# rapidsai/cuvs

Measured on AMD Instinct MI355X. Metric: QPS @ recall@10>=0.9, 100Mx128 fp32 IVF-PQ, batch=10k, higher is better.
Workload: dtype u8 codes, f16 LUT, f32 score; 1 GPU; IVF-PQ 100000000x128 fp32, pq_dim=64 pq_bits=8 n_lists=16384 n_probes=128 batch=10000 k=10; rows and held-out queries from bench.gen_rows (seed 1234 / 4321): Gaussian mixture of 65536 modes ~ N(0, I) in a 32-d latent space, spread 0.35 per mode, embedded in R^128 by a fixed random map + N(0, 0.03^2 I) - NOT SURVEY 8d's generator: the same step on that one is the top-level entry contract_corpus (--; parallelism=single GPU, lut_dtype=f16, internal_distance_dtype=f32

## Files before the change

cuvs_amd/csrc/common.hpp:

```cpp
#pragma once

#include <hip/hip_runtime.h>
#include <hip/hip_fp16.h>

#include <dlpack/dlpack.h>

#include <cstdarg>
#include <cstdint>
#include <cstdio>
#include <cstring>
#include <memory>
#include <stdexcept>
#include <string>
#include <chrono>
#include <vector>

namespace cuvs_amd {

struct error : public std::runtime_error {
  explicit error(const std::string& s) : std::runtime_error(s) {}
};

[[noreturn]] inline void fail(const char* file, int line, const char* fmt, ...)
{
// ... 15 lines not shown
#define HIP_TRY(expr)                                                                        \
  do {                                                                                       \
    hipError_t e__ = (expr);                                                                 \
    if (e__ != hipSuccess) {                                                                 \
      ::cuvs_amd::fail(__FILE__, __LINE__, "HIP error %d (%s) in %s", (int)e__,              \
                       hipGetErrorString(e__), #expr);                                       \
    }                                                                                        \
  } while (0)

std::string& last_error_text();

template <typename Fn>
int translate_exceptions(Fn&& fn)
{
  try {
    fn();
    return 1;
  } catch (const std::exception& e) {
    last_error_text() = e.what();
    return 0;
  } catch (...) {
    last_error_text() = "unknown exception";
    return 0;
  }
}

struct tuning {
  int pq_head_probes    = -1;
  int pq_scan2          = 1;
  int pq_scan3          = 1;
  int coarse_lowp       = 1;
  int pq_head_rows      = -1;
  int pq_overlap        = 1;
  int coarse_grouped    = 1;
  int pq_filter4        = 1;
  int flat_scan3        = 1;
  int flat_filter2      = 1;
  int flat_bound_head   = 1;
  int pq_wide           = 1;
  int pq_wide_heads     = 0;
  int pq_wide_blocks    = 1;
  bool pq_encode_plain  = false;
  int pq3_surv_cap      = 0;
  int pq_qcap           = 0;
  int scan_debug        = 0;
  int alloc_cache       = 1;
  bool shard_coarse_replicated = false;
  bool bf_fused = false, bf_no_threshold = false, bf_no_fused_filter = false;
  bool bf_host_flags = false;
  bool dist_old         = false;
  int tile_dbg          = 0;
  int flat_head_probes  = -1;
  int cagra_pq_lists = 0, cagra_pq_probes = 0, cagra_kpq = 0, cagra_rank_chunk = 0, prune_dbg = 0;
  bool cagra_auto_multi = false;
  int tiered_path       = 0;
  bool native_format    = false;
};
tuning load_tuning_from_env();

struct resources {
  tuning tune;
  int device              = 0;
  hipStream_t stream      = nullptr;
  bool owns_stream        = false;
  int num_cus             = 256;
  size_t lds_per_block    = 160 * 1024;
// ... 211 lines not shown
```

cuvs_amd/csrc/core.hip:

```cpp
#include <cuvs/version_config.h>
#include "common.hpp"

#include <cuvs/core/c_api.h>

#include "scratch_cache.hpp"

#include <algorithm>
#include <cstdlib>
#include <mutex>
#include <vector>

namespace cuvs_amd {

std::string& last_error_text()
{
  thread_local std::string text;
  return text;
}

namespace {

void* raw_alloc(resources& res, size_t bytes, bool* failed)
{
  void* p = nullptr;
  hipError_t e = res.pool != nullptr ? hipMallocFromPoolAsync(&p, bytes, res.pool, res.stream)
                                     : hipMallocAsync(&p, bytes, res.stream);
  if (e != hipSuccess) {
    (void)hipGetLastError();
    if (failed != nullptr) { *failed = true; return nullptr; }
    HIP_TRY(hipStreamSynchronize(res.stream));
    HIP_TRY(hipMalloc(&p, bytes));
  }
  return p;
}

void raw_free(void* stream_v, void* p)
{
  hipStream_t stream = static_cast<hipStream_t>(stream_v);
  hipError_t e = hipFreeAsync(p, stream);
  if (e != hipSuccess) {
    (void)hipGetLastError();
    (void)hipStreamSynchronize(stream);
    (void)hipFree(p);
  }
}

}

unsigned long long g_pq3_last_stats[6] = {0, 0, 0, 0, 0, 0};

static void flush_cache(scratch_cache& c)
{
  if (!c.caller_stream) { c.flush(raw_free); return; }
  bool drained = false;
  c.flush([&](void*, void* p) {
    if (!drained) { (void)hipDeviceSynchronize(); drained = true; }
    (void)hipFree(p);
    (void)hipGetLastError();
  });
}
void scratch_cache_flush(resources& res)
{
  if (res.cache != nullptr) flush_cache(*res.cache);
}

namespace {
std::mutex g_caches_mu;
std::vector<scratch_cache*> g_caches;
}
void scratch_cache_register(scratch_cache* c, bool add)
{
  std::lock_guard<std::mutex> lk(g_caches_mu);
  if (add) g_caches.push_back(c);
  else g_caches.erase(std::remove(g_caches.begin(), g_caches.end(), c), g_caches.end());
}
void scratch_cache_flush_all()
{
  {
    std::lock_guard<std::mutex> lk(g_caches_mu);
    for (scratch_cache* c : g_caches) flush_cache(*c);
  }
  (void)hipDeviceSynchronize();
// ... 63 lines not shown
  g_prof.push_back(r);
}
void profile_end(resources& res, const char* name)
{
  if (!g_prof_on) return;
  std::lock_guard<std::mutex> lk(g_prof_mu);
  for (auto it = g_prof.rbegin(); it != g_prof.rend(); ++it)
    if (it->name == name) { HIP_TRY(hipEventRecord(it->stop, res.stream)); return; }
}

static bool debug_switches_on()
{
#ifdef CUVS_AMD_NO_DEBUG_SWITCHES
  return false;
#else
  const char* g = getenv("CUVS_AMD_DEBUG_SWITCHES");
  return g != nullptr && g[0] == '1';
#endif
}

tuning load_tuning_from_env()
{
  tuning t;
  if (!debug_switches_on()) return t;
  auto geti = [](const char* name, int dflt) { const char* e = getenv(name); return e ? atoi(e) : dflt; };
  auto set  = [](const char* name) { return getenv(name) != nullptr; };
  t.pq_head_probes   = geti("CUVS_AMD_PQ_HEAD_PROBES", -1);
  t.pq_scan2         = geti("CUVS_AMD_PQ_SCAN2", 1);
  t.pq_scan3         = geti("CUVS_AMD_PQ_SCAN3", 1);
  t.pq_filter4       = geti("CUVS_AMD_PQ_FILTER4", 1);
  t.coarse_grouped   = geti("CUVS_AMD_COARSE_GROUPED", 1);
  t.pq_overlap       = geti("CUVS_AMD_PQ_OVERLAP", 1);
  t.pq_head_rows     = geti("CUVS_AMD_PQ_HEAD_ROWS", -1);
  t.coarse_lowp      = geti("CUVS_AMD_COARSE_LOWP", 1);
  t.flat_scan3       = geti("CUVS_AMD_FLAT_SCAN3", 1);
  t.flat_filter2     = geti("CUVS_AMD_FLAT_FILTER2", 1);
  t.flat_bound_head  = geti("CUVS_AMD_FLAT_BOUND_HEAD", 1);
  t.pq_wide          = geti("CUVS_AMD_PQ_WIDE", 1);
  t.pq_wide_heads    = geti("CUVS_AMD_PQ_WIDE_HEADS", 0);
  t.pq_wide_blocks   = geti("CUVS_AMD_PQ_WIDE_BLOCKS", 1);
  if (const char* e = getenv("CUVS_AMD_PQ_ENCODE")) t.pq_encode_plain = strcmp(e, "plain") == 0;
  t.pq3_surv_cap     = geti("CUVS_AMD_PQ3_SURV_CAP", 0);
  t.pq_qcap          = geti("CUVS_AMD_PQ_QCAP", 0);
  t.scan_debug       = geti("CUVS_AMD_SCAN_DEBUG", 0);
  t.alloc_cache      = geti("CUVS_AMD_ALLOC_CACHE", 1);
  t.shard_coarse_replicated = set("CUVS_AMD_SHARD_COARSE_REPLICATED");
  t.bf_fused           = set("CUVS_AMD_BF_FUSED");
  t.bf_no_threshold    = set("CUVS_AMD_BF_NO_THRESHOLD");
  t.bf_no_fused_filter = set("CUVS_AMD_BF_NO_FUSED_FILTER");
  t.bf_host_flags = set("CUVS_AMD_BF_HOST_FLAGS");
  t.dist_old           = set("CUVS_AMD_DIST_OLD");
  t.tile_dbg           = geti("CUVS_AMD_TILE_DBG", 0);
  t.flat_head_probes   = geti("CUVS_AMD_FLAT_HEAD_PROBES", -1);
  t.cagra_pq_lists     = geti("CUVS_AMD_CAGRA_PQ_LISTS", 0);
  t.cagra_pq_probes    = geti("CUVS_AMD_CAGRA_PQ_PROBES", 0);
  t.cagra_kpq          = geti("CUVS_AMD_CAGRA_KPQ", 0);
  t.cagra_rank_chunk   = geti("CUVS_AMD_CAGRA_RANK_CHUNK", 0);
  t.prune_dbg          = geti("CUVS_AMD_PRUNE_DBG", 0);
  if (const char* e = getenv("CUVS_AMD_CAGRA_AUTO")) t.cagra_auto_multi = e[0] == 'm';
  if (const char* e = getenv("CUVS_AMD_TIERED_PATH")) t.tiered_path = strcmp(e, "composed") == 0 ? 1 : (strcmp(e, "fused") == 0 ? 2 : 0);
  if (const char* e = getenv("CUVS_AMD_NATIVE_FORMAT")) t.native_format = e[0] == '1';
  return t;
}

}

// ... 201 lines not shown
}

cuvsError_t cuvsRMMMemoryResourceReset() { return CUVS_SUCCESS; }

cuvsError_t cuvsRMMHostAlloc(void** ptr, size_t bytes)
{
  return (cuvsError_t)translate_exceptions([=] {
    CUVS_EXPECTS(ptr != nullptr, "ptr is null");
    HIP_TRY(hipHostMalloc(ptr, bytes, hipHostMallocDefault));
  });
}

cuvsError_t cuvsRMMHostFree(void* ptr, size_t)
{
  return (cuvsError_t)translate_exceptions([=] { HIP_TRY(hipHostFree(ptr)); });
}

__attribute__((visibility("default"))) int cuvsAmdDebugSwitchesCompiledIn(void)
{
#ifdef CUVS_AMD_NO_DEBUG_SWITCHES
  return 0;
#else
  return 1;
#endif
}
__attribute__((visibility("default"))) void cuvsAmdIvfPqLastFilterStats(unsigned long long* out)
{
  for (int i = 0; i < 4; ++i) out[i] = cuvs_amd::g_pq3_last_stats[i];
}
__attribute__((visibility("default"))) void cuvsAmdIvfPqLastFilterStats6(unsigned long long* out)
{
  for (int i = 0; i < 6; ++i) out[i] = cuvs_amd::g_pq3_last_stats[i];
}
__attribute__((visibility("default"))) void cuvsAmdProfileEnable(int on) { g_prof_on = on != 0; }
__attribute__((visibility("default"))) int cuvsAmdProfileCollect(const char* name, double* total_ms)
{
  std::lock_guard<std::mutex> lk(g_prof_mu);
  int count = 0;
  double total = 0;
  std::vector<prof_rec> keep;
  for (auto& r : g_prof) {
    if (r.name == name) {
      if (hipEventSynchronize(r.stop) == hipSuccess) {
        float ms = 0;
        if (hipEventElapsedTime(&ms, r.start, r.stop) == hipSuccess) { total += ms; ++count; }
      }
      (void)hipEventDestroy(r.start);
      (void)hipEventDestroy(r.stop);
    } else {
      keep.push_back(r);
    }
  }
  g_prof.swap(keep);
  if (total_ms) *total_ms = total;
  return count;
}

cuvsError_t cuvsVersionGet(uint16_t* major, uint16_t* minor, uint16_t* patch)
{
  return (cuvsError_t)translate_exceptions([=] {
    CUVS_EXPECTS(major && minor && patch, "null output");
    *major = CUVS_VERSION_MAJOR; *minor = CUVS_VERSION_MINOR; *patch = CUVS_VERSION_PATCH;
  });
}

cuvsError_t cuvsMatrixCopy(cuvsResources_t res, DLManagedTensor* src_m, DLManagedTensor* dst_m)
// ... 46 lines not shown
```

cuvs_amd/csrc/ivf_pq_scan3.hip:

```cpp
#include "ivf_pq.hpp"
#include "ops.hpp"
#include "device_utils.hpp"
#include "ivf_common.hpp"
#include "pq_lut_math.hpp"
#include "ivf_pq_scan3.hpp"
#include "ivf_pq_filter_common.hpp"

#include <cfloat>
#include <cmath>
#include <cstring>
#include <mutex>
#include <type_traits>

namespace cuvs_amd {

namespace {

constexpr int kFThreads = 512;
constexpr int kFWaves   = kFThreads / 64;



__global__ void cb16_kernel(const float* __restrict__ pq_centers, uint32_t pq_dim, uint32_t pq_len, uint32_t book, float sc,
                            uint16_t* __restrict__ cb16)
// ... 1767 lines not shown
            } else {
              const float t = qq[e] - x[e4 * 4 + e];
              acc = __fmaf_rn(t, t, acc);
            }
          }
        }
      }
    }
    if (a.is_ip == 2) acc = acc / (sqrtf(qn2) * sqrtf(xn2));
    pool_append_wave(a, ok, q, pair, row, a.is_ip ? -acc : acc);
  }
}

struct head_params {
  const work_item* items;
  const uint32_t* item_begin;
  const uint32_t* item_end;
  uint32_t n_lists;
  uint32_t* xcd_ticket;
  const uint32_t* sorted_pairs;
  const float* rot_queries;
  const float* centers_rot;
  const float* pq_centers;
  const uint8_t* codes;
  const uint32_t* list_offsets;
  const uint32_t* list_sizes;
  float* out_d;
  uint32_t* out_i;
  uint32_t* query_kth;
  uint32_t n_probes, rot_dim, k, cap_rows, pq_dim, n_chunks, pq_len, book;
  int is_ip, per_cluster;
  int hcand;
  uint32_t row_limit;
  uint32_t one_shot;
  const uint32_t* filter_bits;
  const int64_t* indices;
  unsigned long long* stats;
};

static inline int head_cand(int k) { return k <= 128 ? 512 : 1024; }

template <int LUT, bool ACC_HALF, int NT>
__global__ __launch_bounds__(NT) __attribute__((amdgpu_waves_per_eu(4, 4))) void pq_head_kernel(const head_params a)
{
  constexpr bool LUT32 = LUT == 0 || (LUT == 2 && !ACC_HALF);
  using lut_t = std::conditional_t<LUT32, float, _Float16>;
  extern __shared__ __attribute__((aligned(16))) char smem[];
  lut_t* lut      = reinterpret_cast<lut_t*>(smem);
  float* rv       = reinterpret_cast<float*>(smem + (size_t)a.pq_dim * 256 * sizeof(lut_t));
  float* cv       = rv + 256;
  unsigned long long* min64 = reinterpret_cast<unsigned long long*>(cv + 256);
  int* ctrl       = reinterpret_cast<int*>(min64 + 2);
  work_item& cur  = *reinterpret_cast<work_item*>(ctrl + 8);
  uint32_t* tk    = reinterpret_cast<uint32_t*>(ctrl + 12);
  const int kHCand = a.hcand;
  uint2* cand     = reinterpret_cast<uint2*>(tk + NT);
  uint32_t* keys  = reinterpret_cast<uint32_t*>(cand + 2 * kHCand);
  static_assert(sizeof(work_item) == 16, "work_item");

  const int tid = threadIdx.x;
  const uint32_t item0   = (a.one_shot == 0u && a.item_begin) ? *a.item_begin : 0u;
  const uint32_t n_items = a.one_shot != 0u ? a.one_shot : *a.item_end - item0;
  const uint32_t xcd = blockIdx.x & 7u, chunk = (n_items + 7u) / 8u;
  const uint32_t share0 = min(n_items, xcd * chunk), share_len = min(chunk, n_items - share0);
  const work_item* share = a.items + item0 + share0;
  const uint4* codes16   = reinterpret_cast<const uint4*>(a.codes);
// ... 74 lines not shown
            p[j] = a.pq_centers[(size_t)((a.per_cluster ? L : sb) * a.pq_len + l) * a.book + code];
          }
#pragma unroll
          for (int j = 0; j < 4; ++j) {
            const uint32_t e = min(e0 + (uint32_t)j * NT, a.pq_dim * 256u - 1u), dd = (e >> 8) * a.pq_len + l;
            const float qv = rv[dd];
            if (!a.is_ip) {
              const float d = qv - p[j];
              v[j] = __fmaf_rn(d, d, v[j]);
            } else {
              v[j] = __fmaf_rn(-qv, cv[dd], v[j]);
              v[j] = __fmaf_rn(-qv, p[j], v[j]);
            }
          }
        }
#pragma unroll
        for (int j = 0; j < 4; ++j) {
          const uint32_t e = e0 + (uint32_t)j * NT;
          if (e >= a.pq_dim * 256u) break;
          float x = v[j];
          if constexpr (LUT == 2) x = fp8_round_trip<std::conditional_t<ACC_HALF, __half, float>>(x, a.is_ip != 0);
          if constexpr (LUT32) lut[e] = x; else lut[e] = to_lut_half(x);
        }
      }
    }
    if (tid == 0) ctrl[0] = 0;
    __syncthreads();
    phase(1);
    const int k = (int)a.k;
    int buf = 0;
    for (uint32_t c0 = 0; c0 < len; c0 += a.cap_rows) {
      const uint32_t clen = min(a.cap_rows, len - c0);
      uint32_t my_min = 0xffffffffu;
      for (uint32_t v = tid; v < clen; v += NT) {
        const uint32_t fr = base_row + c0 + v;
        const uint4* cp   = codes16 + ((size_t)(fr >> 6) * a.n_chunks) * 64 + (fr & 63u);
        float af    = 0.f;
        _Float16 ah = (_Float16)0.f;
        for (int c0c = 0; c0c < (int)a.n_chunks; c0c += 4) {
          uint4 cw[4];
#pragma unroll
          for (int c = 0; c < 4; ++c) cw[c] = cp[(size_t)min(c0c + c, (int)a.n_chunks - 1) * 64];
#pragma unroll
          for (int cc = 0; cc < 4; ++cc) {
            const int c = c0c + cc;
            if (c >= (int)a.n_chunks) break;
            const uint32_t ws[4] = {cw[cc].x, cw[cc].y, cw[cc].z, cw[cc].w};
            lut_t e[16];
#pragma unroll
            for (int b = 0; b < 16; ++b) e[b] = lut[((c * 16 + b) << 8) + ((ws[b >> 2] >> ((b & 3) * 8)) & 0xffu)];
            __builtin_amdgcn_sched_barrier(0);
#pragma unroll
            for (int b = 0; b < 16; ++b) {
              if constexpr (LUT32) af += e[b];
              else if constexpr (ACC_HALF) ah += e[b];
              else af += (float)e[b];
            }
          }
        }
        const float score = ACC_HALF ? (float)ah : af;
        bool keep = true;
        if (a.filter_bits != nullptr) {
          const int64_t sid = a.indices[fr];
          keep = ((a.filter_bits[sid >> 5] >> (sid & 31)) & 1u) != 0u;
        }
        const uint32_t key = keep ? float_to_key(score) : 0xffffffffu;
        keys[v] = key;
        my_min  = min(my_min, key);
      }
      const int gshift = k > 128 ? 0 : (k > 64 ? 1 : 2);
      if (gshift >= 1)
        my_min = min(my_min, (uint32_t)__builtin_amdgcn_update_dpp((int)my_min, (int)my_min, 0xb1, 0xf, 0xf, false));
      if (gshift == 2)
        my_min = min(my_min, (uint32_t)__builtin_amdgcn_update_dpp((int)my_min, (int)my_min, 0x4e, 0xf, 0xf, false));
      if ((tid & ((1 << gshift) - 1)) == 0) tk[tid >> gshift] = my_min;
      __syncthreads();
      phase(2);
      const int NGr   = NT >> gshift;
      const int k_c   = (int)min((uint32_t)k, clen);
      const int kept  = ctrl[0];
      if (tid < NGr) {
        const uint32_t mine = tk[tid];
        const uint4* tk4    = reinterpret_cast<const uint4*>(tk);
        int r = 0;
#pragma unroll 4
        for (int j = 0; j < NGr / 4; ++j) {
          const uint4 o = tk4[j];
          r += (o.x < mine || (o.x == mine && 4 * j + 0 < tid)) ? 1 : 0;
          r += (o.y < mine || (o.y == mine && 4 * j + 1 < tid)) ? 1 : 0;
          r += (o.z < mine || (o.z == mine && 4 * j + 2 < tid)) ? 1 : 0;
          r += (o.w < mine || (o.w == mine && 4 * j + 3 < tid)) ? 1 : 0;
        }
        if (r == k_c - 1) ctrl[1] = (int)mine;
        if (tid == 0) ctrl[2] = kept;
      }
      __syncthreads();
      const uint32_t tau = (uint32_t)ctrl[1];
      uint2* bc = cand + buf * kHCand;
      for (uint32_t i = tid; i < clen; i += NT) {
        const uint32_t key = keys[i];
        if (key <= tau && key != 0xffffffffu) {
          const int pos = atomicAdd(&ctrl[2], 1);
          if (pos < kHCand) bc[pos] = make_uint2(key, c0 + i);
        }
      }
      __syncthreads();
      int cnt = ctrl[2];
      if (cnt > kHCand) {
        unsigned long long last = 0ull;
        bool first = true;
        cnt = kept;
// ... 450 lines not shown
  hipLaunchKernelGGL(reset_flagged_kernel, dim3((unsigned)r.nq), dim3(256), 0, res.stream, r.qflag, r.nq, r.n_probes, r.k, r.head,
                     r.cand_d, r.cand_i);
  hipLaunchKernelGGL(fallback_items_kernel, dim3(grid * 4), dim3(256), 0, res.stream, r.sorted_pairs, r.pair_off, idx.n_lists,
                     r.probes, r.n_probes, r.qflag, static_cast<work_item*>(r.fb_items), r.counters, 0);
  profile_end(res, "pq_scan_kernel");
}

static size_t head_smem_fixed(const ivf_pq_index& idx, int lut_mode, bool acc_half, int nt, int k)
{
  const bool lut32 = lut_mode == 0 || (lut_mode == 2 && !acc_half);
  return (size_t)idx.pq_dim * 256 * (lut32 ? 4 : 2) + 2 * 256 * 4 + 16 + 32 + 16 + (size_t)nt * 4 + 4 * (size_t)head_cand(k) * 4;
}

void pq3_head_scan(resources& res, const ivf_pq_index& idx, const pq3_head& h)
{
  head_params a{};
  a.items = static_cast<const work_item*>(h.items); a.item_begin = h.item_begin; a.item_end = h.item_end; a.n_lists = idx.n_lists;
  a.xcd_ticket = h.xcd_ticket; a.sorted_pairs = h.sorted_pairs; a.rot_queries = h.rot_queries; a.centers_rot = idx.centers_rot.data();
  a.pq_centers = idx.pq_centers.data(); a.codes = pq3_codes(res, idx, &a.n_chunks); a.list_offsets = idx.list_offsets.data();
  a.list_sizes = idx.list_sizes.data(); a.out_d = h.cand_d; a.out_i = h.cand_i; a.query_kth = h.query_kth;
  a.n_probes = h.n_probes; a.rot_dim = idx.rot_dim; a.k = h.k; a.is_ip = h.is_ip; a.pq_dim = idx.pq_dim;
  a.pq_len = idx.pq_len; a.book = idx.pq_book; a.per_cluster = idx.codebook_kind != 0 ? 1 : 0;
  a.filter_bits = h.filter_bits; a.indices = idx.indices.data(); a.stats = h.stats; a.hcand = head_cand((int)h.k);
  const bool lut32 = h.lut_mode == 0 || (h.lut_mode == 2 && !h.acc_half);
  const bool small = (size_t)idx.pq_dim * 256 * (lut32 ? 4 : 2) <= 32 * 1024;
  const int nt = small ? 512 : 1024;
  const size_t budget = (small ? 80 : 160) * 1024 - 64, fixed = head_smem_fixed(idx, h.lut_mode, h.acc_half != 0, nt, (int)h.k);
  CUVS_EXPECTS(budget > fixed + 4096, "ivf_pq: the head-phase LUT does not fit the LDS");
  a.cap_rows = (uint32_t)(((budget - fixed) / 4) & ~size_t(63));
  if (h.max_list_len > 0) a.cap_rows = std::min<uint32_t>(a.cap_rows, (uint32_t)round_up(h.max_list_len, 64));
  const size_t smem   = fixed + (size_t)a.cap_rows * 4;
  a.one_shot          = h.one_shot;
  a.row_limit         = h.row_limit;
  const unsigned grid = h.one_shot != 0u ? h.one_shot : pq3_grid(res) * (small ? 2u : 1u);
  auto go = [&](auto kern) {
    HIP_TRY(hipFuncSetAttribute(reinterpret_cast<const void*>(kern), hipFuncAttributeMaxDynamicSharedMemorySize, (int)smem));
    profile_begin(res, "pq_scan_kernel");
    profile_begin(res, "pq_head_kernel");
    hipLaunchKernelGGL(kern, dim3(grid), dim3(nt), smem, res.stream, a);
    profile_end(res, "pq_head_kernel");
    profile_end(res, "pq_scan_kernel");
  };
  auto pick = [&](auto lut_tag, auto acc_tag) {
    constexpr int LUT = decltype(lut_tag)::value;
    constexpr bool ACC = decltype(acc_tag)::value;
    if (small) go(pq_head_kernel<LUT, ACC, 512>); else go(pq_head_kernel<LUT, ACC, 1024>);
  };
  using I0 = std::integral_constant<int, 0>; using I1 = std::integral_constant<int, 1>; using I2 = std::integral_constant<int, 2>;
  if (h.lut_mode == 0)      pick(I0{}, std::false_type{});
  else if (h.lut_mode == 1) { if (h.acc_half) pick(I1{}, std::true_type{}); else pick(I1{}, std::false_type{}); }
  else                      { if (h.acc_half) pick(I2{}, std::true_type{}); else pick(I2{}, std::false_type{}); }
}

bool flat3_wide(uint32_t dim) { return dim > 128 && pqw_shape(dim); }
bool flat3_supported(uint32_t dim, int k) { return ((dim % 32 == 0 && dim >= 32 && dim <= 256) || flat3_wide(dim)) && k <= 128; }

static bool flat3_prepare(resources& res, const flat3_view& v, flat3_cache& c)
{
  static std::mutex mu;
  std::lock_guard<std::mutex> lock(mu);
  if (c.data_ptr == v.data && c.rows == v.padded_rows && c.size == v.size) return true;
  if (c.failed_ptr == v.data && c.failed_rows == v.padded_rows && c.failed_size == v.size) return false;
  const int64_t rows = std::max<int64_t>(v.padded_rows, 64);
  {
    c.rows16   = dev_buf<uint4>();
    c.row_term = dev_buf<uint32_t>();
// ... 461 lines not shown
```

cuvs_amd/csrc/ivf_pq_search.hip:

```cpp
#include "ivf_pq.hpp"
#include "ops.hpp"
#include "device_utils.hpp"
#include "ivf_common.hpp"
#include "pq_lut_math.hpp"
#include "ivf_pq_scan3.hpp"

#include <cuvs/neighbors/ivf_pq.h>

#include <cfloat>
#include <cstdlib>
#include <functional>
#include <mutex>
#include <type_traits>

namespace cuvs_amd {
extern unsigned long long g_pq3_last_stats[6];

void load_range_as_float(resources& res, const void* data, elem_t et, bool is_host, int64_t dim, int64_t r0,
                         int64_t cnt, float* out);

namespace {

constexpr int kScanThreads = 1024;
constexpr int kScanWaves   = kScanThreads / 64;
constexpr int kQueueRows   = 320;

inline unsigned nblk(int64_t n, int per) { return grid_blocks(n, per); }

template <typename LutT, typename AccT, int QPB>
struct lut_acc;

typedef float f32x2_t __attribute__((ext_vector_type(2)));
typedef float f32x4_t __attribute__((ext_vector_type(4)));
typedef _Float16 f16x2_t __attribute__((ext_vector_type(2)));
typedef _Float16 f16x4_t __attribute__((ext_vector_type(4)));

template <>
struct lut_acc<float, float, 1> {
  using entry_t = float;
  float a       = 0.f;
  __device__ inline void add(entry_t e) { a += e; }
  __device__ inline float get(int) const { return a; }
  __device__ static inline entry_t pack(const float (&v)[1]) { return v[0]; }
};
template <>
struct lut_acc<float, float, 2> {
  using entry_t = f32x2_t;
  f32x2_t a     = {0.f, 0.f};
  __device__ inline void add(entry_t e) { a += e; }
// ... 1952 lines not shown
    w_x = dev_buf<float>(res, w ? bs * pl.wheads * pl.w_ldx : 0); w_kv = dev_buf<float>(res, w ? bs * k : 0);
    w_thr = dev_buf<float>(res, wh); w_c = dev_buf<float>(res, wh);
    w_ki = dev_buf<uint32_t>(res, w ? bs * k : 0); w_blk = dev_buf<uint32_t>(res, w ? nl + 1 : 0);
    w_bt = dev_buf<uint32_t>(res, w ? 2 * bs : 0); w_nm = dev_buf<float4>(res, wh);
    hitems = dev_buf<work_item>(res, ov ? bs : 0); hpairs = dev_buf<uint32_t>(res, ov ? bs + 1 : 0);
    pair_norms = dev_buf<float4>(res, ov ? np : 0); group_scratch = dev_buf<uint32_t>(res, ov ? np + pl.n_labels + 1 : 0);
    glut_buf = dev_buf<char>(res, pl.glut_stride * pl.grid);
    stats = dev_buf<unsigned long long>(res, (res.tune.scan_debug & (128 | 512)) ? (size_t)ST_COUNT * pl.grid * kScanWaves : 0);
  }
};

struct aux_fork_guard {
  hipStream_t s = nullptr;
  bool armed    = false;
  ~aux_fork_guard() { if (armed && s != nullptr) (void)hipStreamSynchronize(s); }
};

struct pq_search_ctx {
  resources& res;
  resources& gres;
  const ivf_pq_search_params& p;
  const ivf_pq_index& idx;
  const pq_search_plan& pl;
  pq_search_scratch& s;
  aux_fork_guard& fork_guard;
  int k;
  const uint32_t* filter_bits;
};

void report_head_stats(resources& res, const unsigned long long* d_stats)
{
  auto hs = to_host(res, d_stats, 8);
  const double n = (double)std::max<unsigned long long>(1, hs[5]);
  fprintf(stderr, "[pq_head] items %llu; workgroup cycles per item: header %.0f, LUT %.0f, scores %.0f, select %.0f, output %.0f\n", hs[5],
          hs[0] / n, hs[1] / n, hs[2] / n, hs[3] / n, hs[4] / n);
}

void report_filter_stats(resources& res, const unsigned long long* d_stats, const uint32_t* counters)
{
  auto hs = to_host(res, d_stats, 8);
  g_pq3_last_stats[0] = hs[0]; g_pq3_last_stats[1] = hs[1]; g_pq3_last_stats[2] = hs[2]; g_pq3_last_stats[3] = hs[7];
  fprintf(stderr, "[pq_scan3] units %llu; wave cycles per unit: prologue %.0f, loop %.0f (slow path %.0f); per subtile %.0f\n", hs[7],
          (double)hs[4] / std::max<unsigned long long>(1, hs[7]), (double)hs[5] / std::max<unsigned long long>(1, hs[7]),
          (double)hs[6] / std::max<unsigned long long>(1, hs[7]), (double)hs[5] / std::max<unsigned long long>(1, hs[2]));
  auto hc = to_host(res, counters, 2);
  g_pq3_last_stats[4] = hc[0]; g_pq3_last_stats[5] = hc[1];
  fprintf(stderr, "[pq_scan3] overflow entries %u\n", hc[1]);
  hc[1] = hc[0];
  fprintf(stderr, "[pq_scan3] pairs screened %llu, survivors %llu (%.4f%%), subtiles %llu (slow path %llu), fallback pairs %u\n",
          hs[0], hs[1], 100.0 * hs[1] / (double)std::max<unsigned long long>(1, hs[0]), hs[2], hs[3], hc[1]);
}

void report_scan_stats(resources& res, const dev_buf<unsigned long long>& stats, unsigned grid, int dbg)
{
  std::vector<unsigned long long> hw(stats.n);
  HIP_TRY(hipMemcpyAsync(hw.data(), stats.data(), stats.bytes(), hipMemcpyDeviceToHost, res.stream));
  HIP_TRY(hipStreamSynchronize(res.stream));
  unsigned long long h[ST_COUNT] = {};
  for (size_t i = 0; i < hw.size(); ++i) h[i % ST_COUNT] += hw[i];
  const double w = 1.0 / (16.0 * grid);
  if (dbg & 4096) {
    for (int which : {(int)ST_SCAN, (int)ST_ALIVE2, (int)ST_F_GATHER, (int)ST_F_FLUSH, (int)ST_STAGE2, (int)ST_CAND, (int)ST_S2_CALLS}) {
      fprintf(stderr, "[pq_scan per-wave stat %d, Mcycles]", which);
      for (int wv = 0; wv < kScanWaves; ++wv) {
        unsigned long long t = 0;
        for (unsigned b = 0; b < grid; ++b) t += hw[((size_t)b * kScanWaves + wv) * ST_COUNT + which];
        fprintf(stderr, " %.2f", (double)t / grid * 1e-6);
      }
// ... 218 lines not shown
                     distances + q0 * k);
}

}

void ivf_pq_search(resources& res, const ivf_pq_search_params& p, const ivf_pq_index& idx, const void* queries,
                   elem_t et, int64_t n_queries, int k, int64_t* neighbors, float* distances, const uint32_t* filter_bits)
{
  CUVS_EXPECTS(k > 0, "parameter `k` in top-k must be positive.");
  CUVS_EXPECTS((int64_t)k <= idx.size || idx.shard_world > 1,
               "parameter `k` (%d) in top-k must not be larger that the total size of the index (%ld)", k,
               (long)idx.size);
  CUVS_EXPECTS(p.n_probes > 0, "n_probes (number of clusters to probe in the search) must be positive.");
  CUVS_EXPECTS(p.internal_distance_dtype == 0 || p.internal_distance_dtype == 2,
               "internal_distance_dtype must be either CUDA_R_16F or CUDA_R_32F");
  CUVS_EXPECTS(p.lut_dtype == 0 || p.lut_dtype == 2 || p.lut_dtype == 8 || p.lut_dtype == 3,
               "lut_dtype must be CUDA_R_16F, CUDA_R_32F, CUDA_R_8U or CUDA_R_8I");
  CUVS_EXPECTS(p.coarse_search_dtype == 0 || p.coarse_search_dtype == 2 || p.coarse_search_dtype == 3,
               "Unsupported coarse_search_dtype (only CUDA_R_32F, CUDA_R_16F, and CUDA_R_8I are supported)");
  CUVS_EXPECTS(!idx.dtype_known || et == idx.dtype, "queries dtype differs from the index dtype");
  if (n_queries == 0) return;
  if (idx.shard_comm != nullptr && !idx.shard_stats_valid) shard_exchange_stats(res, idx);
  const bool large_k   = k > 256;
  size_t largest_total = large_k ? largest_lists_total(idx.h_list_sizes, std::min<uint32_t>(p.n_probes, idx.n_lists)) : 0;
  if (large_k && idx.shard_comm != nullptr) {
    dev_buf<uint32_t> key(res, 1);
    const uint32_t mine = ~(uint32_t)std::min<size_t>(largest_total, 0xfffffffeu);
    copy_async(res, key.data(), &mine, sizeof(mine));
    shard_allreduce_min_u32(res, idx.shard_comm, key.data(), 1);
    largest_total = (size_t)~to_host(res, key.data(), 1)[0];
  }
  const pq_search_plan pl = make_pq_search_plan(idx, p, k, n_queries, res.tune, res.num_cus, res.ivf_batch_limit, largest_total,
                                                [&] { return pqw_ready(res, idx); });
  if (res.tune.scan_debug & 1024)
    fprintf(stderr, "[pq_wide] heads %u (supported %d, matrix-core tail of the narrow shapes %d, probes %u, queries %ld, k %d)\n", pl.wheads,
            (int)pqw_supported(idx, k), (int)(pq3_supported(idx, k) && pq3_bound_useful(idx, k)), pl.n_probes, (long)n_queries, k);
  pq_search_scratch scratch(res, idx, p, pl, k);
  resources aux = res;
  if (pl.overlap) {
    ensure_aux_stream(res);
    aux.aux_stream = res.aux_stream;
    aux.stream     = res.aux_stream;
  }
  aux_fork_guard fork_guard;
  fork_guard.s = pl.overlap ? aux.stream : nullptr;
  const pq_search_ctx c{res, pl.overlap ? aux : res, p, idx, pl, scratch, fork_guard, k, filter_bits};
  for (int64_t q0 = 0; q0 < n_queries; q0 += pl.max_batch)
    pq_search_batch(c, queries, et, q0, std::min(pl.max_batch, n_queries - q0), neighbors, distances);
  HIP_TRY(hipGetLastError());
}

}

extern "C" __attribute__((visibility("default"))) int cuvsAmdIvfPqSearchPlan(
  uint32_t dim, uint32_t rot_dim, uint32_t pq_dim, uint32_t pq_len, uint32_t pq_bits, uint32_t shard_world, int codebook_kind,
  int metric, uint32_t n_lists, const uint32_t* list_sizes, cuvsIvfPqSearchParams_t params, int k, int64_t n_queries, int num_cus,
  uint64_t batch_limit_bytes, int wide_rows_ready, int64_t out[24])
{
  return cuvs_amd::translate_exceptions([=] {
    using namespace cuvs_amd;
    CUVS_EXPECTS(params != nullptr && list_sizes != nullptr && n_lists > 0 && pq_bits >= 4 && pq_bits <= 8, "invalid argument");
    ivf_pq_index idx;
    idx.metric = metric; idx.codebook_kind = codebook_kind; idx.n_lists = n_lists; idx.dim = dim; idx.rot_dim = rot_dim;
    idx.pq_dim = pq_dim; idx.pq_len = pq_len; idx.pq_bits = pq_bits; idx.pq_book = 1u << pq_bits;
    idx.codes_per_chunk = 128 / pq_bits; idx.n_chunks = (uint32_t)ceil_div(pq_dim, idx.codes_per_chunk);
    idx.shard_world = (int)std::max(1u, shard_world);
// ... 16 lines not shown
```

include/cuvs_amd/extensions.h:

```cpp
#pragma once
#include <cuvs/core/c_api.h>
#include <cuvs/core/export.h>
#include <cuvs/neighbors/all_neighbors.h>
#include <cuvs/neighbors/cagra.h>
#include <cuvs/neighbors/common.h>
#include <cuvs/neighbors/ivf_pq.h>
#include <cuvs/neighbors/tiered_index.h>
#include <cuvs/neighbors/vamana.h>
#include <cuvs/preprocessing/quantize/binary.h>
#include <cuvs/preprocessing/quantize/pq.h>
#include <stdint.h>

#ifdef __cplusplus
extern "C" {
#endif

CUVS_EXPORT cuvsError_t cuvsAmdIvfPqSearchFiltered(cuvsResources_t res, cuvsIvfPqSearchParams_t search_params,
                                                   cuvsIvfPqIndex_t index, DLManagedTensor* queries,
                                                   DLManagedTensor* neighbors, DLManagedTensor* distances,
                                                   cuvsFilter filter);

CUVS_EXPORT cuvsError_t cuvsAmdCagraWorkCounters(cuvsResources_t res, int enable, uint64_t out[3]);

CUVS_EXPORT cuvsError_t cuvsAmdCagraSetGuaranteeConnectivity(cuvsResources_t res, int on);
// ... 28 lines not shown

CUVS_EXPORT cuvsError_t cuvsAmdTieredIndexGetInfo(cuvsTieredIndex_t index, int64_t* size, int64_t* ann_rows, int64_t* capacity,
                                                  int64_t* dim);
CUVS_EXPORT cuvsError_t cuvsAmdTieredIndexCompact(cuvsResources_t res, cuvsTieredIndex_t index);
CUVS_EXPORT cuvsError_t cuvsAmdTieredIndexSearchTiers(cuvsResources_t res, void* search_params, cuvsTieredIndex_t index,
                                                      DLManagedTensor* queries, DLManagedTensor* ann_neighbors,
                                                      DLManagedTensor* ann_distances, DLManagedTensor* tail_neighbors,
                                                      DLManagedTensor* tail_distances, cuvsFilter prefilter);
CUVS_EXPORT cuvsError_t cuvsAmdTieredTailSearch(cuvsResources_t res, cuvsDistanceType metric, DLManagedTensor* tail, int64_t ann_rows,
                                                DLManagedTensor* queries, DLManagedTensor* seed_neighbors,
                                                DLManagedTensor* seed_distances, DLManagedTensor* bitset, int path,
                                                DLManagedTensor* neighbors, DLManagedTensor* distances);
CUVS_EXPORT cuvsError_t cuvsAmdTieredMerge(cuvsResources_t res, DLManagedTensor* a_neighbors, DLManagedTensor* a_distances,
                                           DLManagedTensor* b_neighbors, DLManagedTensor* b_distances, int64_t ann_rows,
                                           int select_min, DLManagedTensor* out_neighbors, DLManagedTensor* out_distances);
CUVS_EXPORT void cuvsAmdTieredCounters(unsigned long long out[3]);

CUVS_EXPORT cuvsError_t cuvsAmdVamanaIndexGetGraph(cuvsResources_t res, cuvsVamanaIndex_t index, DLManagedTensor* out);
CUVS_EXPORT cuvsError_t cuvsAmdVamanaIndexGetMedoid(cuvsVamanaIndex_t index, uint32_t* medoid);
CUVS_EXPORT cuvsError_t cuvsAmdVamanaGreedySearch(cuvsResources_t res, cuvsVamanaIndexParams_t params, DLManagedTensor* dataset,
                                                  DLManagedTensor* graph, uint32_t medoid, DLManagedTensor* query_ids,
                                                  DLManagedTensor* out_ids, DLManagedTensor* out_dists);
CUVS_EXPORT cuvsError_t cuvsAmdVamanaRobustPrune(cuvsResources_t res, cuvsVamanaIndexParams_t params, DLManagedTensor* dataset,
                                                 DLManagedTensor* graph, DLManagedTensor* node_ids, DLManagedTensor* cand_ids,
                                                 DLManagedTensor* cand_dists, DLManagedTensor* out_ids);
CUVS_EXPORT cuvsError_t cuvsAmdVamanaSerializeSectorAligned(cuvsResources_t res, const char* filename, cuvsVamanaIndex_t index,
                                                            bool include_dataset);

CUVS_EXPORT int cuvsAmdDebugSwitchesCompiledIn(void);
CUVS_EXPORT void cuvsAmdProfileEnable(int on);
CUVS_EXPORT int cuvsAmdProfileCollect(const char* name, double* total_ms);
CUVS_EXPORT void cuvsAmdIvfPqLastFilterStats(unsigned long long out[4]);
CUVS_EXPORT void cuvsAmdIvfPqLastFilterStats6(unsigned long long out[6]);

CUVS_EXPORT cuvsError_t cuvsAmdPcaLastSweeps(int* sweeps);

#ifdef __cplusplus
}
#endif
```

Before: 1.819 million queries/s.

## Add early-stop staged scoring in PQ head kernel using seed-derived threshold

In the PQ head kernel, the first 2*NT rows of each chunk are scored fully, and the k-th smallest key among the group minima becomes a pruning threshold. Remaining rows are scored on their first code chunk only. Rows whose partial L2 sum already exceeds the threshold are dropped, and survivors are queued in a per-wave ring in shared memory to finish their remaining chunks. The aim is to skip most LUT lookups for rows that cannot make the top-k, at the cost of extra synchronisation, ring bookkeeping and divergence. Debug statistics counting dropped rows are also added.

```diff
diff --git a/cuvs_amd/csrc/common.hpp b/cuvs_amd/csrc/common.hpp
--- a/cuvs_amd/csrc/common.hpp
+++ b/cuvs_amd/csrc/common.hpp
@@ -71,6 +71,7 @@
   int coarse_lowp       = 1;
   int pq_head_rows      = -1;
   int pq_overlap        = 1;
+  int pq_head_stop      = 1;
   int coarse_grouped    = 1;
   int pq_filter4        = 1;
   int flat_scan3        = 1;
diff --git a/cuvs_amd/csrc/core.hip b/cuvs_amd/csrc/core.hip
--- a/cuvs_amd/csrc/core.hip
+++ b/cuvs_amd/csrc/core.hip
@@ -48,6 +48,7 @@
 }
 
 unsigned long long g_pq3_last_stats[6] = {0, 0, 0, 0, 0, 0};
+unsigned long long g_pq_head_last_stats[8] = {0, 0, 0, 0, 0, 0, 0, 0};
 
 static void flush_cache(scratch_cache& c)
 {
@@ -177,6 +178,7 @@
   t.coarse_grouped   = geti("CUVS_AMD_COARSE_GROUPED", 1);
   t.pq_overlap       = geti("CUVS_AMD_PQ_OVERLAP", 1);
   t.pq_head_rows     = geti("CUVS_AMD_PQ_HEAD_ROWS", -1);
+  t.pq_head_stop     = geti("CUVS_AMD_PQ_HEAD_STOP", 1);
   t.coarse_lowp      = geti("CUVS_AMD_COARSE_LOWP", 1);
   t.flat_scan3       = geti("CUVS_AMD_FLAT_SCAN3", 1);
   t.flat_filter2     = geti("CUVS_AMD_FLAT_FILTER2", 1);
@@ -444,6 +446,10 @@
 {
   for (int i = 0; i < 6; ++i) out[i] = cuvs_amd::g_pq3_last_stats[i];
 }
+__attribute__((visibility("default"))) void cuvsAmdIvfPqLastHeadStats(unsigned long long* out)
+{
+  for (int i = 0; i < 8; ++i) out[i] = cuvs_amd::g_pq_head_last_stats[i];
+}
 __attribute__((visibility("default"))) void cuvsAmdProfileEnable(int on) { g_prof_on = on != 0; }
 __attribute__((visibility("default"))) int cuvsAmdProfileCollect(const char* name, double* total_ms)
 {
diff --git a/cuvs_amd/csrc/ivf_pq_scan3.hip b/cuvs_amd/csrc/ivf_pq_scan3.hip
--- a/cuvs_amd/csrc/ivf_pq_scan3.hip
+++ b/cuvs_amd/csrc/ivf_pq_scan3.hip
@@ -1823,6 +1823,7 @@
   int is_ip, per_cluster;
   int hcand;
   uint32_t row_limit;
+  uint32_t stop;
   uint32_t one_shot;
   const uint32_t* filter_bits;
   const int64_t* indices;
@@ -1963,19 +1964,17 @@
     for (uint32_t c0 = 0; c0 < len; c0 += a.cap_rows) {
       const uint32_t clen = min(a.cap_rows, len - c0);
       uint32_t my_min = 0xffffffffu;
-      for (uint32_t v = tid; v < clen; v += NT) {
-        const uint32_t fr = base_row + c0 + v;
-        const uint4* cp   = codes16 + ((size_t)(fr >> 6) * a.n_chunks) * 64 + (fr & 63u);
-        float af    = 0.f;
-        _Float16 ah = (_Float16)0.f;
-        for (int c0c = 0; c0c < (int)a.n_chunks; c0c += 4) {
+      const int gshift = k > 128 ? 0 : (k > 64 ? 1 : 2);
+      const int NGr    = NT >> gshift;
+      auto add_chunks = [&](const uint4* cp, int cb, int ce, float& af, _Float16& ah) {
+        for (int c0c = cb; c0c < ce; c0c += 4) {
           uint4 cw[4];
 #pragma unroll
-          for (int c = 0; c < 4; ++c) cw[c] = cp[(size_t)min(c0c + c, (int)a.n_chunks - 1) * 64];
+          for (int c = 0; c < 4; ++c) cw[c] = cp[(size_t)min(c0c + c, ce - 1) * 64];
 #pragma unroll
           for (int cc = 0; cc < 4; ++cc) {
             const int c = c0c + cc;
-            if (c >= (int)a.n_chunks) break;
+            if (c >= ce) break;
             const uint32_t ws[4] = {cw[cc].x, cw[cc].y, cw[cc].z, cw[cc].w};
             lut_t e[16];
 #pragma unroll
@@ -1989,17 +1988,116 @@
             }
           }
         }
-        const float score = ACC_HALF ? (float)ah : af;
-        bool keep = true;
-        if (a.filter_bits != nullptr) {
-          const int64_t sid = a.indices[fr];
-          keep = ((a.filter_bits[sid >> 5] >> (sid & 31)) & 1u) != 0u;
-        }
-        const uint32_t key = keep ? float_to_key(score) : 0xffffffffu;
+      };
+      auto row_codes = [&](uint32_t v) {
+        const uint32_t fr = base_row + c0 + v;
+        return codes16 + ((size_t)(fr >> 6) * a.n_chunks) * 64 + (fr & 63u);
+      };
+      auto row_kept = [&](uint32_t v) {
+        if (a.filter_bits == nullptr) return true;
+        const int64_t sid = a.indices[base_row + c0 + v];
+        return ((a.filter_bits[sid >> 5] >> (sid & 31)) & 1u) != 0u;
+      };
+      constexpr uint32_t kSeed = 2u * NT;
+      const bool staged    = a.stop != 0u && !a.is_ip && a.n_chunks >= 2u && clen > kSeed;
+      const uint32_t full  = staged ? kSeed : clen;
+      for (uint32_t v = tid; v < full; v += NT) {
+        float af    = 0.f;
+        _Float16 ah = (_Float16)0.f;
+        add_chunks(row_codes(v), 0, (int)a.n_chunks, af, ah);
+        const float score  = ACC_HALF ? (float)ah : af;
+        const uint32_t key = row_kept(v) ? float_to_key(score) : 0xffffffffu;
         keys[v] = key;
         my_min  = min(my_min, key);
       }
-      const int gshift = k > 128 ? 0 : (k > 64 ? 1 : 2);
+      if (staged) {
+        uint32_t gm = my_min;
+        if (gshift >= 1) gm = min(gm, (uint32_t)__builtin_amdgcn_update_dpp((int)gm, (int)gm, 0xb1, 0xf, 0xf, false));
+        if (gshift == 2) gm = min(gm, (uint32_t)__builtin_amdgcn_update_dpp((int)gm, (int)gm, 0x4e, 0xf, 0xf, false));
+        if ((tid & ((1 << gshift) - 1)) == 0) tk[tid >> gshift] = gm;
+        __syncthreads();
+        if (tid < NGr) {
+          const uint32_t mine = tk[tid];
+          const uint4* tk4    = reinterpret_cast<const uint4*>(tk);
+          int r = 0;
+#pragma unroll 4
+          for (int j = 0; j < NGr / 4; ++j) {
+            const uint4 o = tk4[j];
+            r += (o.x < mine || (o.x == mine && 4 * j + 0 < tid)) ? 1 : 0;
+            r += (o.y < mine || (o.y == mine && 4 * j + 1 < tid)) ? 1 : 0;
+            r += (o.z < mine || (o.z == mine && 4 * j + 2 < tid)) ? 1 : 0;
+            r += (o.w < mine || (o.w == mine && 4 * j + 3 < tid)) ? 1 : 0;
+          }
+          if (r == k - 1) ctrl[3] = (int)mine;
+        }
+        __syncthreads();
+        const float tau_f = key_to_float((uint32_t)ctrl[3]);
+        const uint32_t lane = (uint32_t)tid & 63u;
+        uint16_t* ring = reinterpret_cast<uint16_t*>(cand + (buf ^ 1) * kHCand) + ((uint32_t)tid >> 6) * 128u;
+        uint32_t q_head = 0, q_tail = 0, n_drop = 0;
+        auto finish = [&](uint32_t n) {
+          __builtin_amdgcn_fence(__ATOMIC_ACQ_REL, "wavefront");
+          if (lane < n) {
+            const uint32_t v = ring[(q_head + lane) & 127u];
+            const uint32_t p = keys[v];
+            float af    = 0.f;
+            _Float16 ah = (_Float16)0.f;
+            if constexpr (ACC_HALF) ah = __builtin_bit_cast(_Float16, (uint16_t)p); else af = __uint_as_float(p);
+            add_chunks(row_codes(v), 1, (int)a.n_chunks, af, ah);
+            const uint32_t key = float_to_key(ACC_HALF ? (float)ah : af);
+            keys[v] = key;
+            my_min  = min(my_min, key);
+          }
+          q_head += n;
+        };
+        uint4 nw[4];
+        auto first_chunks = [&](uint32_t v0) {
+#pragma unroll
+          for (int j = 0; j < 4; ++j) {
+            const uint32_t vj = v0 + (uint32_t)j * NT;
+            nw[j] = vj < clen ? *row_codes(vj) : make_uint4(0u, 0u, 0u, 0u);
+          }
+        };
+        first_chunks(kSeed + tid);
+        for (uint32_t v0 = kSeed + tid; v0 - lane < clen; v0 += 4u * NT) {
+          const uint4 w0 = nw[0], w1 = nw[1], w2 = nw[2], w3 = nw[3];
+          first_chunks(v0 + 4u * NT);
+#pragma unroll 1
+          for (uint32_t j = 0; j < 4u && v0 + j * NT - lane < clen; ++j) {
+            const uint32_t v = v0 + j * NT;
+            const bool in = v < clen;
+            const uint4 w = j == 0u ? w0 : (j == 1u ? w1 : (j == 2u ? w2 : w3));
+            const uint32_t ws[4] = {w.x, w.y, w.z, w.w};
+            lut_t e[16];
+#pragma unroll
+            for (int b = 0; b < 16; ++b) e[b] = lut[(b << 8) + ((ws[b >> 2] >> ((b & 3) * 8)) & 0xffu)];
+            __builtin_amdgcn_sched_barrier(0);
+            float af    = 0.f;
+            _Float16 ah = (_Float16)0.f;
+#pragma unroll
+            for (int b = 0; b < 16; ++b) {
+              if constexpr (LUT32) af += e[b];
+              else if constexpr (ACC_HALF) ah += e[b];
+              else af += (float)e[b];
+            }
+            const bool valid = in && row_kept(v);
+            const bool drop  = valid && (ACC_HALF ? (float)ah : af) > tau_f;
+            const bool live  = valid && !drop;
+            const unsigned long long m = __ballot(live);
+            if (in) keys[v] = live ? (ACC_HALF ? (uint32_t)__builtin_bit_cast(uint16_t, ah) : __float_as_uint(af)) : 0xffffffffu;
+            if (live) {
+              const uint32_t pos = __builtin_amdgcn_mbcnt_hi((uint32_t)(m >> 32), __builtin_amdgcn_mbcnt_lo((uint32_t)m, 0u));
+              ring[(q_tail + pos) & 127u] = (uint16_t)v;
+            }
+            q_tail += (uint32_t)__popcll(m);
+            n_drop += (uint32_t)__popcll(__ballot(drop));
+            if (q_tail - q_head >= 64u) finish(64u);
+          }
+        }
+        if (q_tail != q_head) finish(q_tail - q_head);
+        if (a.stats != nullptr && lane == 0u) atomicAdd(&a.stats[6], (unsigned long long)n_drop);
+      }
+      if (a.stats != nullptr && tid == 0) atomicAdd(&a.stats[7], (unsigned long long)clen);
       if (gshift >= 1)
         my_min = min(my_min, (uint32_t)__builtin_amdgcn_update_dpp((int)my_min, (int)my_min, 0xb1, 0xf, 0xf, false));
       if (gshift == 2)
@@ -2007,7 +2105,6 @@
       if ((tid & ((1 << gshift) - 1)) == 0) tk[tid >> gshift] = my_min;
       __syncthreads();
       phase(2);
-      const int NGr   = NT >> gshift;
       const int k_c   = (int)min((uint32_t)k, clen);
       const int kept  = ctrl[0];
       if (tid < NGr) {
@@ -2524,6 +2621,7 @@
   const size_t smem   = fixed + (size_t)a.cap_rows * 4;
   a.one_shot          = h.one_shot;
   a.row_limit         = h.row_limit;
+  a.stop              = res.tune.pq_head_stop != 0 ? 1u : 0u;
   const unsigned grid = h.one_shot != 0u ? h.one_shot : pq3_grid(res) * (small ? 2u : 1u);
   auto go = [&](auto kern) {
     HIP_TRY(hipFuncSetAttribute(reinterpret_cast<const void*>(kern), hipFuncAttributeMaxDynamicSharedMemorySize, (int)smem));
diff --git a/cuvs_amd/csrc/ivf_pq_search.hip b/cuvs_amd/csrc/ivf_pq_search.hip
--- a/cuvs_amd/csrc/ivf_pq_search.hip
+++ b/cuvs_amd/csrc/ivf_pq_search.hip
@@ -15,6 +15,7 @@
 
 namespace cuvs_amd {
 extern unsigned long long g_pq3_last_stats[6];
+extern unsigned long long g_pq_head_last_stats[8];
 
 void load_range_as_float(resources& res, const void* data, elem_t et, bool is_host, int64_t dim, int64_t r0,
                          int64_t cnt, float* out);
@@ -2033,8 +2034,10 @@
 {
   auto hs = to_host(res, d_stats, 8);
   const double n = (double)std::max<unsigned long long>(1, hs[5]);
-  fprintf(stderr, "[pq_head] items %llu; workgroup cycles per item: header %.0f, LUT %.0f, scores %.0f, select %.0f, output %.0f\n", hs[5],
-          hs[0] / n, hs[1] / n, hs[2] / n, hs[3] / n, hs[4] / n);
+  fprintf(stderr, "[pq_head] items %llu; workgroup cycles per item: header %.0f, LUT %.0f, scores %.0f, select %.0f, output %.0f; rows "
+          "scored %llu, dropped after their first code chunk %llu (%.1f%%)\n", hs[5], hs[0] / n, hs[1] / n, hs[2] / n, hs[3] / n, hs[4] / n,
+          hs[7], hs[6], 100.0 * hs[6] / (double)std::max<unsigned long long>(1, hs[7]));
+  for (int i = 0; i < 8; ++i) g_pq_head_last_stats[i] += hs[i];
 }
 
 void report_filter_stats(resources& res, const unsigned long long* d_stats, const uint32_t* counters)
@@ -2319,6 +2322,8 @@
   }
   const pq_search_plan pl = make_pq_search_plan(idx, p, k, n_queries, res.tune, res.num_cus, res.ivf_batch_limit, largest_total,
                                                 [&] { return pqw_ready(res, idx); });
+  if (res.tune.scan_debug & 2048)
+    for (auto& v : g_pq_head_last_stats) v = 0;
   if (res.tune.scan_debug & 1024)
     fprintf(stderr, "[pq_wide] heads %u (supported %d, matrix-core tail of the narrow shapes %d, probes %u, queries %ld, k %d)\n", pl.wheads,
             (int)pqw_supported(idx, k), (int)(pq3_supported(idx, k) && pq3_bound_useful(idx, k)), pl.n_probes, (long)n_queries, k);
diff --git a/include/cuvs_amd/extensions.h b/include/cuvs_amd/extensions.h
--- a/include/cuvs_amd/extensions.h
+++ b/include/cuvs_amd/extensions.h
@@ -84,6 +84,7 @@
 CUVS_EXPORT int cuvsAmdProfileCollect(const char* name, double* total_ms);
 CUVS_EXPORT void cuvsAmdIvfPqLastFilterStats(unsigned long long out[4]);
 CUVS_EXPORT void cuvsAmdIvfPqLastFilterStats6(unsigned long long out[6]);
+CUVS_EXPORT void cuvsAmdIvfPqLastHeadStats(unsigned long long out[8]);
 
 CUVS_EXPORT cuvsError_t cuvsAmdPcaLastSweeps(int* sweeps);
 
```

Result: no change. 1.832 million queries/s, median of 6 (+0.7%).
